# TengdaHan/DPC

Hardware: AMD Instinct MI355X
Metric: clips/sec (train step, B x8x3x5xHxW) (higher is better)
Workload: dtype bf16; 1 GPU; cfg2: resnet18 2d3d, img_dim 128, seq_len 5, num_seq 8, pred_step 3, batch 128/GPU, full train step (fwd+CE/top-k+bwd+all-reduce+Adam); global_batch=128, parallelism=dp1, init=reference init, random, launch=hipGraph replay, streams=2

## Files before the change

dpc_amd/csrc/conv_igemm_ws.hip:

```cpp
#include "conv_common.h"
#include <stdlib.h>

struct WsParams {
    GatherGeom g;
    const void* src;
    const void* wgt;
    void* out;
    const void* addend;
    float* stats;
    int Ncol, ldw, ldo;
    int gm, ntn, ntm;
    unsigned src_bytes, wgt_bytes;
    int tgroup, hw, nclip, tpt, cpkt;
    FastDiv d_hw;
    int plane;
    int parity;
    ParityInfo par;
    int dbg;
};
#ifdef DPC_WS_PROBE
#define WS_DBG(bit) (p.dbg & (bit))
#else
#define WS_DBG(bit) 0
#endif

#include "ws_frag.h"

template <bool HAS_ADD, bool PAR = false>
__global__ __launch_bounds__(512, 2) void igemm_ws_kernel(WsParams p) {
    typedef bf16_t T;
    typedef bf16_t TO;
    constexpr int BM = 256, BN = 128, BKE = 64;
    constexpr int STAGE = (BM + BN) * 128;
    constexpr int NST = 3;
    constexpr int EPO = 8, UPR = BN / EPO;
    __shared__ __attribute__((aligned(1024))) unsigned char lds[NST * STAGE];

    const GatherGeom& g = p.g;
    const int tid = threadIdx.x;
    const int lane = tid & 63;
#ifdef DPC_SIMT_EMU
    const int wv = tid >> 6;
#else
    const int wv = __builtin_amdgcn_readfirstlane(tid >> 6);
#endif
    const int n_tile = blockIdx.x / p.gm;
    const int m_prog = blockIdx.x % p.gm;
    const int nkc = g.Kp / BKE;
    const int my_tiles = (p.ntm - m_prog + p.gm - 1) / p.gm;
    struct ParCls { int j, rows, ct, ch, cw, Tc, Hc, Wc; FastDiv dT, dH, dW; };
    auto par_cls = [&](int mt) -> ParCls {
        ParCls k;
        int c;
        parity_tile(p.par, mt, c, k.j);
        k.cw = c & (g.sw - 1); k.ch = (c >> g.lsw) & (g.sh - 1); k.ct = c >> (g.lsw + g.lsh);
        k.Tc = k.ct ? p.par.dimc[0][1] : p.par.dimc[0][0]; k.dT = k.ct ? p.par.div[0][1] : p.par.div[0][0];
        k.Hc = k.ch ? p.par.dimc[1][1] : p.par.dimc[1][0]; k.dH = k.ch ? p.par.div[1][1] : p.par.div[1][0];
        k.Wc = k.cw ? p.par.dimc[2][1] : p.par.dimc[2][0]; k.dW = k.cw ? p.par.div[2][1] : p.par.div[2][0];
        k.rows = p.par.N * k.Tc * k.Hc * k.Wc;
        return k;
    };
    auto par_decode = [&](const ParCls& k, int lr, int& n, int& tq, int& hq, int& wq) {
        const unsigned q1 = fdiv((unsigned)lr, k.dW);
        wq = lr - (int)q1 * k.Wc;
        const unsigned q2 = fdiv(q1, k.dH);
        hq = (int)q1 - (int)q2 * k.Hc;
        const unsigned nn = fdiv(q2, k.dT);
        tq = (int)q2 - (int)nn * k.Tc;
        n = (int)nn;
    };
    auto par_row = [&](const ParCls& k, int r) -> int {
        const int lr = k.j * BM + r;
        if (lr >= k.rows) return g.M;
        int n, tq, hq, wq;
        par_decode(k, lr, n, tq, hq, wq);
        return (((n * g.RT + tq * g.st + k.ct) * g.RH + hq * g.sh + k.ch) * g.RW) + wq * g.sw + k.cw;
    };
    auto par_pk = [&](const ParCls& k, unsigned& pT, unsigned& pH, unsigned& pW) {
        pT = k.ct ? p.par.pk[0][1] : p.par.pk[0][0];
        pH = k.ch ? p.par.pk[1][1] : p.par.pk[1][0];
        pW = k.cw ? p.par.pk[2][1] : p.par.pk[2][0];
    };
    auto tile_row = [&](int mt, int r) -> int {
        if (!p.tgroup) return mt * BM + r;
        const int t = mt / p.tpt;
        const unsigned idx = (unsigned)((mt - t * p.tpt) * BM + r);
        const unsigned clip = fdiv(idx, p.d_hw);
        return (int)clip < p.nclip ? (int)((clip * (unsigned)g.RT + (unsigned)t) * (unsigned)p.hw + (idx - clip * (unsigned)p.hw)) : g.M;
    };
    auto tile_chunks = [&](int mt, int& lo, int& hi) {
        lo = 0; hi = nkc;
        if (PAR) {
            const ParCls k = par_cls(mt);
            unsigned pT, pH, pW;
            par_pk(k, pT, pH, pW);
            hi = par_pk_n(pT) * par_pk_n(pH) * par_pk_n(pW) * (g.Ci >> 6);
            return;
        }
        if (!p.tgroup) return;
        const int t = mt / p.tpt;
        int klo, khi;
        if (g.mode == 0) { klo = g.pt - t; khi = g.ST - 1 + g.pt - t; }
        else { klo = t + g.pt - (g.ST - 1); khi = t + g.pt; }
        if (klo < 0) klo = 0;
        if (khi > g.KT - 1) khi = g.KT - 1;
        lo = klo * p.cpkt; hi = (khi + 1) * p.cpkt;
    };
    int total = 0;
    for (int t = 0; t < my_tiles; ++t) {
        int lo, hi;
        tile_chunks(m_prog + t * p.gm, lo, hi);
        total += hi - lo;
    }
    const char* const zero = (const char*)dpc_zero16;

    if (wv >= 4) {
        const int lw = wv - 4;
        const int rl = lane >> 3;
        const int u = (lane & 7) ^ lds_swz1(8 * lw + rl);
        const BufRsrc rs_a = make_buf_rsrc(p.src, p.src_bytes);
        const BufRsrc rs_b = make_buf_rsrc(p.wgt, p.wgt_bytes);
        unsigned wrow[4];
        DPC_UNROLL
        for (int i = 0; i < 4; ++i) {
            const int n = n_tile * BN + 8 * (lw + 4 * i) + rl;
            wrow[i] = n < p.Ncol ? (unsigned)(n * p.ldw + u * 8) * 2u : DPC_BUF_OOB;
        }
        unsigned rowoff[8];
        unsigned vmask[8];
        auto range_bits = [](int x0, int sgn, int K, int S) -> unsigned {
            int lo, hi;
            if (sgn > 0) { lo = -x0; hi = S - 1 - x0; } else { lo = x0 - S + 1; hi = x0; }
            if (lo < 0) lo = 0;
            if (hi > K - 1) hi = K - 1;
            return hi >= lo ? (((2u << hi) - 1u) & ~((1u << lo) - 1u)) : 0u;
        };
        unsigned l_pT = 0, l_pH = 0, l_pW = 0;
        int l_jt = 0, l_jh = 0, l_jw = 0, l_cc = 0;
        auto decode_tile = [&](int mt) {
            const int mine = lane & 7;
            if (PAR) {
                const ParCls k = par_cls(mt);
                par_pk(k, l_pT, l_pH, l_pW);
                l_jt = l_jh = l_jw = l_cc = 0;
                const int lr = k.j * BM + 8 * (lw + 4 * mine) + rl;
                unsigned off = 0, m = 0;
                if (lr < k.rows) {
                    int n, tq, hq, wq;
                    par_decode(k, lr, n, tq, hq, wq);
                    off = (((((unsigned)(n * g.ST + tq) * (unsigned)g.SH + (unsigned)hq) * (unsigned)g.SW) + (unsigned)wq) * (unsigned)g.src_ld) * 2u;
                    DPC_UNROLL
                    for (int j = 0; j < 4; ++j) {
                        m |= (j < par_pk_n(l_pT) && (unsigned)(tq + par_pk_dl(l_pT, j)) < (unsigned)g.ST ? 1u : 0u) << j;
                        m |= (j < par_pk_n(l_pH) && (unsigned)(hq + par_pk_dl(l_pH, j)) < (unsigned)g.SH ? 1u : 0u) << (4 + j);
                        m |= (j < par_pk_n(l_pW) && (unsigned)(wq + par_pk_dl(l_pW, j)) < (unsigned)g.SW ? 1u : 0u) << (8 + j);
                    }
                }
                DPC_UNROLL
                for (int i = 0; i < 8; ++i) {
                    const int from = (lane & ~7) | i;
                    rowoff[i] = (unsigned)__shfl((int)off, from) + (unsigned)(u * 16);
                    vmask[i] = (unsigned)__shfl((int)m, from);
                }
                return;
            }
            const RowPos rp = decode_row(g, tile_row(mt, 8 * (lw + 4 * mine) + rl));
            const unsigned off = (((((unsigned)(rp.nbase + rp.t0) * (unsigned)g.SH + (unsigned)rp.h0) * (unsigned)g.SW) + (unsigned)rp.w0) *
                                  (unsigned)g.src_ld) * 2u;
            const int sgn = g.mode == 0 ? 1 : -1;
            const unsigned m = range_bits(rp.t0, sgn, g.KT, g.ST) | (range_bits(rp.h0, sgn, g.KH, g.SH) << g.KT) |
                               (range_bits(rp.w0, sgn, g.KW, g.SW) << (g.KT + g.KH));
            DPC_UNROLL
            for (int i = 0; i < 8; ++i) {
                const int from = (lane & ~7) | i;
                rowoff[i] = (unsigned)__shfl((int)off, from) + (unsigned)(u * 16);
                vmask[i] = (unsigned)__shfl((int)m, from);
            }
        };
        auto issue = [&](int kc, int stage) {
            unsigned char* st = lds + stage * STAGE;
            if (PAR) {
                const int jt = l_jt, jh = l_jh, jw = l_jw, cofs = l_cc * BKE;
                if (++l_cc == (g.Ci >> 6)) {
                    l_cc = 0;
                    if (++l_jw == par_pk_n(l_pW)) {
                        l_jw = 0;
                        if (++l_jh == par_pk_n(l_pH)) { l_jh = 0; ++l_jt; }
                    }
                }
                const int kt = par_pk_kl(l_pT, jt), kh = par_pk_kl(l_pH, jh), kw = par_pk_kl(l_pW, jw);
                const int dt = par_pk_dl(l_pT, jt), dh = par_pk_dl(l_pH, jh), dw = par_pk_dl(l_pW, jw);
                const unsigned sel = (1u << jt) | (1u << (4 + jh)) | (1u << (8 + jw));
                const unsigned tapoff = (unsigned)(((dt * g.SH + dh) * g.SW + dw) * g.src_ld + cofs) * 2u;
                const unsigned kd = (unsigned)(((kt * g.KH + kh) * g.KW + kw) * g.Ci + cofs);
                DPC_UNROLL
                for (int i = 0; i < 8; ++i) {
                    const bool ok = (vmask[i] & sel) == sel;
                    if (!WS_DBG(4 | 128)) glds16_buf(rs_a, ok ? rowoff[i] + tapoff : DPC_BUF_OOB, 0u, st + (lw + 4 * i) * 1024, lane);
                }
                DPC_UNROLL
                for (int i = 0; i < 4; ++i)
                    if (!WS_DBG(4 | 256)) glds16_buf(rs_b, wrow[i], kd * 2u, st + BM * 128 + (lw + 4 * i) * 1024, lane);
                return;
            }
            const int kd = kc * BKE;
            const int tap = (g.taps == 1) ? 0 : (kd >> g.log2C);
            const unsigned q = fdiv((unsigned)tap, g.dKW);
            const int kw = tap - (int)q * g.KW;
            const unsigned kt = fdiv(q, g.dKH);
            const int kh = (int)q - (int)kt * g.KH;
            const unsigned sel = (1u << kt) | (1u << (g.KT + kh)) | (1u << (g.KT + g.KH + kw));
            const int sgn = g.mode == 0 ? 1 : -1;
            const int cbase = (g.taps == 1) ? 0 : (tap << g.log2C);
            const unsigned tapoff = (unsigned)(sgn * ((((int)kt * g.SH + kh) * g.SW + kw) * g.src_ld) + (kd - cbase)) * 2u;
            DPC_UNROLL
            for (int i = 0; i < 8; ++i) {
                const bool ok = (vmask[i] & sel) == sel;
                if (!WS_DBG(4 | 128)) glds16_buf(rs_a, ok ? rowoff[i] + tapoff : DPC_BUF_OOB, 0u, st + (lw + 4 * i) * 1024, lane);
            }
            DPC_UNROLL
            for (int i = 0; i < 4; ++i)
                if (!WS_DBG(4 | 256)) glds16_buf(rs_b, wrow[i], (unsigned)kd * 2u, st + BM * 128 + (lw + 4 * i) * 1024, lane);
        };
        int it_tile = 0, it_kc = 0, it_hi = 0;
        bool it_new = true;
        auto issue_next = [&](int gc) {
            if (it_new) {
                const int mt = m_prog + it_tile * p.gm;
                decode_tile(mt);
                tile_chunks(mt, it_kc, it_hi);
                it_new = false;
            }
            issue(it_kc, gc % NST);
            if (++it_kc == it_hi) { it_new = true; ++it_tile; }
        };
        if (total > 0) issue_next(0);
        if (total > 1) issue_next(1);
        int kc_done = 0, cur_tile = 0, cur_n;
        {
            int lo, hi;
            tile_chunks(m_prog, lo, hi);
            cur_n = hi - lo;
        }
        for (int gc = 0; gc < total; ++gc) {
            if (gc + 1 < total) wait_vmcnt<12>(); else wait_vmcnt<0>();
            ws_barrier();
            if (gc + 2 < total) issue_next(gc + 2);
            if (++kc_done == cur_n) {
                kc_done = 0;
                ws_barrier();
                if (++cur_tile < my_tiles) {
                    int lo, hi;
                    tile_chunks(m_prog + cur_tile * p.gm, lo, hi);
                    cur_n = hi - lo;
                }
            }
        }
    }

    const int l31 = lane & 31, lhi = lane >> 5;
    const ldsa_t lds0 = ldsa(lds);
    const int fa0 = lds_unit_off(wv * 64 + l31, lhi);
    const int fb0 = BM * 128 + lds_unit_off(l31, lhi);
    const int cu = lane & 15, er = lane >> 4;
    const int col0 = n_tile * BN + cu * EPO;
    float s1[EPO], s2[EPO];
    DPC_UNROLL
    for (int e = 0; e < EPO; ++e) { s1[e] = 0.f; s2[e] = 0.f; }

    int gc = 0;
#ifndef DPC_SIMT_EMU
    __builtin_amdgcn_s_setprio(3);
#endif
    for (int t = 0; wv < 4 && t < my_tiles; ++t) {
        const int mt = m_prog + t * p.gm;
        ParCls ck = {};
        if (PAR) ck = par_cls(mt);
        int kc_lo, kc_hi;
        tile_chunks(mt, kc_lo, kc_hi);
        const int nkc_t = kc_hi - kc_lo;
        f32x16 acc[2][4];
        DPC_UNROLL
        for (int i = 0; i < 2; ++i)
            DPC_UNROLL
            for (int j = 0; j < 4; ++j)
                DPC_UNROLL
                for (int r = 0; r < 16; ++r) acc[i][j][r] = 0.f;
        u32x4 av0[8], av1[8];
        auto fetch_addend = [&](int i, u32x4 (&dst)[8]) {
            DPC_UNROLL
            for (int it = 0; it < 8; ++it) {
                const int row = PAR ? par_row(ck, wv * 64 + i * 32 + er + 4 * it) : tile_row(mt, wv * 64 + i * 32 + er + 4 * it);
                const bool ok = row < g.M && col0 < p.Ncol;
                const char* a = (const char*)p.addend + ((long long)row * p.ldo + col0) * 2;
                dst[it] = *(const u32x4*)(ok ? a : (const char*)p.addend);
            }
        };
        int stage_last = 0;
        {
            FragSet f0, f1;
            ws_barrier();
            ldsa_t pa = lds0 + (gc % NST) * STAGE + fa0, pb = lds0 + (gc % NST) * STAGE + fb0;
            frag_read_p2<4096>(f0, pa, pb);
            for (int kc = 0; kc < nkc_t; ++kc) {
                if (HAS_ADD && kc + 1 == nkc_t) fetch_addend(0, av0);
                step_il<true, 4096>(acc, f0, f1, pa ^ 32, pb ^ 32);
                step_il<true, 4096>(acc, f1, f0, pa ^ 64, pb ^ 64);
                step_il<true, 4096>(acc, f0, f1, pa ^ 96, pb ^ 96);
                frag_wait<0>(f1);
                ws_barrier();
                stage_last = gc % NST;
                ++gc;
                pa = lds0 + (gc % NST) * STAGE + fa0;
                pb = lds0 + (gc % NST) * STAGE + fb0;
                step_il<true, 4096>(acc, f1, f0, pa, pb);
            }
            WS_RETIRE_TAIL_READS(f0);
        }

        if (WS_DBG(2)) {
            if (acc[0][0][0] == 12345.f) *(float*)p.out = acc[1][3][5];
            continue;
        }
        unsigned char* mine = lds + stage_last * STAGE + wv * WS_STG_WAVE;
        DPC_UNROLL
        for (int i = 0; i < 2; ++i) {
            stage_block(mine, acc[i], l31, lhi);
            wave_lds_fence();
            if (HAS_ADD && i == 0) fetch_addend(1, av1);
            u32x4 ov[8];
            DPC_UNROLL
            for (int it = 0; it < 8; ++it) {
                const int row_l = er + 4 * it;
                ov[it] = *(const u32x4*)(mine + row_l * WS_STG_ROW + cu * EPO * 2);
            }
            wave_lds_fence();
            DPC_UNROLL
            for (int it = 0; it < 8; ++it) {
                const int row = PAR ? par_row(ck, wv * 64 + i * 32 + er + 4 * it) : tile_row(mt, wv * 64 + i * 32 + er + 4 * it);
                if (row < g.M && col0 < p.Ncol) {
                    u32x4 o = ov[it];
                    if (HAS_ADD) {
                        const u32x4 a = i == 0 ? av0[it] : av1[it];
                        float sv[EPO];
                        DPC_UNROLL
                        for (int e = 0; e < EPO; ++e) sv[e] = unit_get<TO>(o, e) + unit_get<TO>(a, e);
                        o = unit_pack<TO>(sv);
                    }
                    *(u32x4*)((char*)p.out + ((long long)row * p.ldo + col0) * 2) = o;
                    if (!HAS_ADD) {
                        DPC_UNROLL
                        for (int e = 0; e < EPO; ++e) {
                            const float v = unit_get<TO>(o, e);
                            s1[e] += v;
                            s2[e] += v * v;
                        }
                    }
                }
            }
        }
    }

    if (!HAS_ADD && p.stats) {
        DPC_UNROLL
        for (int e = 0; e < EPO; ++e) {
            s1[e] += __shfl_xor(s1[e], 16); s1[e] += __shfl_xor(s1[e], 32);
            s2[e] += __shfl_xor(s2[e], 16); s2[e] += __shfl_xor(s2[e], 32);
        }
        float* red = (float*)lds;
        __syncthreads();
        if (wv < 4 && lane < 16) {
            DPC_UNROLL
            for (int e = 0; e < EPO; ++e) {
                red[(wv * 2 + 0) * BN + cu * EPO + e] = s1[e];
                red[(wv * 2 + 1) * BN + cu * EPO + e] = s2[e];
            }
        }
        __syncthreads();
        if (tid < BN) {
            const int col = n_tile * BN + tid;
            if (col < p.Ncol) {
                float a = 0.f, b = 0.f;
                DPC_UNROLL
                for (int w = 0; w < 4; ++w) {
                    a += red[(w * 2 + 0) * BN + tid];
                    b += red[(w * 2 + 1) * BN + tid];
                }
                p.stats[((long long)m_prog * 2 + 0) * p.Ncol + col] = a;
                p.stats[((long long)m_prog * 2 + 1) * p.Ncol + col] = b;
            }
        }
    }
}


template <bool HAS_ADD>
__global__ __launch_bounds__(512, 2) void igemm_wsp_kernel(WsParams p) {
    typedef bf16_t TO;
    constexpr int BM = 256, BN = 128;
    constexpr int PWD = 18, NPP = PWD * PWD, NPIECE = (NPP + 7) / 8, PATCH = NPIECE * 1024;
    constexpr int BST = BN * 128, NSB = 4;
    constexpr int EPO = 8;
    constexpr int MAXP = (NPIECE + 3) / 4;
    static_assert(4 * WS_STG_WAVE <= PATCH, "epilogue staging fits a patch buffer");
    static_assert(2 * PATCH + NSB * BST <= 160 * 1024, "patches + ring fit the CU's LDS");
    __shared__ __attribute__((aligned(1024))) unsigned char lds[2 * PATCH + NSB * BST];
    unsigned char* const bring = lds + 2 * PATCH;

    const GatherGeom& g = p.g;
    const int tid = threadIdx.x;
    const int lane = tid & 63;
#ifdef DPC_SIMT_EMU
    const int wv = tid >> 6;
#else
    const int wv = __builtin_amdgcn_readfirstlane(tid >> 6);
#endif
    const int n_tile = blockIdx.x / p.gm;
    const int m_prog = blockIdx.x % p.gm;
    const int G = g.Ci >> 6;
    const int nkc = 9 * G;
    const int my_tiles = (p.ntm - m_prog + p.gm - 1) / p.gm;
    const int total = my_tiles * nkc;
    const char* const zero = (const char*)dpc_zero16;

    if (wv >= 4) {
        const int lw = wv - 4;
        const int rl = lane >> 3;
        const BufRsrc rs_a = make_buf_rsrc(p.src, p.src_bytes);
        const BufRsrc rs_b = make_buf_rsrc(p.wgt, p.wgt_bytes);
        const int ub = (lane & 7) ^ lds_swz1(8 * lw + rl);
        unsigned wrow[4];
        DPC_UNROLL
        for (int i = 0; i < 4; ++i) {
            const int n = n_tile * BN + 8 * (lw + 4 * i) + rl;
            wrow[i] = n < p.Ncol ? (unsigned)(n * p.ldw + ub * 8) * 2u : DPC_BUF_OOB;
        }
        unsigned poff[MAXP];
        DPC_UNROLL
        for (int i = 0; i < MAXP; ++i) {
            const int pp = 8 * (lw + 4 * i) + rl;
            const int pr = pp / PWD, pc = pp - pr * PWD;
            const bool ok = pp < NPP && pr >= 1 && pr <= 16 && pc >= 1 && pc <= 16;
            const int up = (lane & 7) ^ ((pc >> 1) & 7);
            poff[i] = ok ? (unsigned)((((pr - 1) * 16 + (pc - 1)) * g.src_ld + up * 8) * 2) : DPC_BUF_OOB;
        }
        const int n_mine = (NPIECE - lw + 3) / 4;
        int issued = 0;
        auto issue_patch = [&](int gg, int i0, int i1) {
            const int tl = gg / G, grp = gg - tl * G;
            const int mt = WS_DBG(512) ? m_prog & 7 : m_prog + tl * p.gm;
            const unsigned soff = (unsigned)((mt * BM * g.src_ld + grp * 64) * 2);
            unsigned char* dst = lds + (gg & 1) * PATCH;
            DPC_UNROLL
            for (int i = 0; i < MAXP; ++i)
                if (i >= i0 && i < i1 && i < n_mine && !WS_DBG(4 | 128)) {
                    glds16_buf(rs_a, poff[i], soff, dst + (lw + 4 * i) * 1024, lane);
                    ++issued;
                }
        };
        auto issue_b = [&](int gc) {
            const int gg = gc / 9, tap = gc - gg * 9;
            const int grp = gg % G;
            const int kd = tap * g.Ci + grp * 64;
            unsigned char* st = bring + (gc % NSB) * BST;
            if (WS_DBG(4 | 256)) return;
            DPC_UNROLL
            for (int i = 0; i < 4; ++i) glds16_buf(rs_b, wrow[i], (unsigned)kd * 2u, st + (lw + 4 * i) * 1024, lane);
            issued += 4;
        };
        if (total > 0) {
            issue_patch(0, 0, MAXP);
            issue_b(0);
        }
        issued = 0;
        if (total > 1) issue_b(1);
        int o2 = issued;
        issued = 0;
        if (total > 2) issue_b(2);
        int o1 = issued;
        for (int gc = 0; gc < total; ++gc) {
            wait_vmcnt_upto(o1 + o2);
            if (!WS_DBG(32)) ws_barrier();
            const int gg = gc / 9, q = gc - gg * 9;
            issued = 0;
            if (q < (MAXP + 1) / 2 && (gg + 1) * 9 < total) issue_patch(gg + 1, 2 * q, 2 * q + 2);
            if (gc + 3 < total) issue_b(gc + 3);
            o2 = o1;
            o1 = issued;
            if (q == 8 && (gg + 1) % G == 0) if (!WS_DBG(32)) ws_barrier();
        }
    }

    const int l31 = lane & 31, lhi = lane >> 5;
    int va[3];
    {
        const int pos0 = ((wv * 64 + l31) >> 4) * PWD + (l31 & 15);
        DPC_UNROLL
        for (int kw = 0; kw < 3; ++kw) {
            const int dw = g.mode == 0 ? kw : 2 - kw;
            const int p7 = (((l31 & 15) + dw) >> 1) & 7;
            va[kw] = (pos0 + dw) * 128 + ((lhi ^ p7) << 4);
        }
    }
    const ldsa_t lds0 = ldsa(lds);
    const int vb = lds_unit_off(l31, lhi);
    const int cu = lane & 15, er = lane >> 4;
    const int col0 = n_tile * BN + cu * EPO;
    float s1[EPO], s2[EPO];
    DPC_UNROLL
    for (int e = 0; e < EPO; ++e) { s1[e] = 0.f; s2[e] = 0.f; }

    int gc = 0;
#ifndef DPC_SIMT_EMU
    __builtin_amdgcn_s_setprio(3);
#endif
    for (int t = 0; wv < 4 && t < my_tiles; ++t) {
        const int mt = m_prog + t * p.gm;
        f32x16 acc[2][4];
        DPC_UNROLL
        for (int i = 0; i < 2; ++i)
            DPC_UNROLL
            for (int j = 0; j < 4; ++j)
                DPC_UNROLL
                for (int r = 0; r < 16; ++r) acc[i][j][r] = 0.f;
        u32x4 av0[8], av1[8];
        auto fetch_addend = [&](int i, u32x4 (&dst)[8]) {
            DPC_UNROLL
            for (int it = 0; it < 8; ++it) {
                const int row = mt * BM + wv * 64 + i * 32 + er + 4 * it;
                const bool ok = row < g.M && col0 < p.Ncol;
                const char* a = (const char*)p.addend + ((long long)row * p.ldo + col0) * 2;
                dst[it] = *(const u32x4*)(ok ? a : (const char*)p.addend);
            }
        };
        {
            FragSet f0, f1;
            if (!WS_DBG(32)) ws_barrier();
            ldsa_t a_row = lds0 + ((t * G) & 1) * PATCH + (g.mode == 0 ? 0 : 2) * (PWD * 128);
            ldsa_t b_st = lds0 + 2 * PATCH + (gc % NSB) * BST;
            ldsa_t pa = a_row + va[0];
            ldsa_t pb = b_st + vb;
            frag_read_p2<4608>(f0, pa, pb);
            for (int gk = 0; gk < 3 * G; ++gk) {
                const int grp = gk / 3, kh = gk - grp * 3;
                const bool last_gk = gk + 1 == 3 * G;
                const int kh_n = kh == 2 ? 0 : kh + 1, gg_n = t * G + (kh == 2 ? grp + 1 : grp);
                const ldsa_t a_row_n = lds0 + (gg_n & 1) * PATCH + (g.mode == 0 ? kh_n : 2 - kh_n) * (PWD * 128);
                static_for<3>([&](auto KWc) {
                    constexpr int KW = decltype(KWc)::value;
                    const bool last = last_gk && KW == 2;
                    if (HAS_ADD && last) fetch_addend(0, av0);
                    step_il<true, 4608>(acc, f0, f1, pa ^ 32, pb ^ 32);
                    step_il<true, 4608>(acc, f1, f0, pa ^ 64, pb ^ 64);
                    step_il<true, 4608>(acc, f0, f1, pa ^ 96, pb ^ 96);
                    frag_wait<0>(f1);
                    if (!WS_DBG(32)) ws_barrier();
                    ++gc;
                    b_st = lds0 + 2 * PATCH + (gc % NSB) * BST;
                    if (KW == 2) a_row = a_row_n;
                    pa = a_row + va[(KW + 1) % 3];
                    pb = b_st + vb;
                    step_il<true, 4608>(acc, f1, f0, pa, pb);
                });
            }
            WS_RETIRE_TAIL_READS(f0);
        }

        unsigned char* mine = lds + ((t * G + G - 1) & 1) * PATCH + wv * WS_STG_WAVE;
        if (WS_DBG(2)) {
            if (acc[0][0][0] == 12345.f) *(float*)p.out = acc[1][3][5];
            continue;
        }
        DPC_UNROLL
        for (int i = 0; i < 2; ++i) {
            stage_block(mine, acc[i], l31, lhi);
            wave_lds_fence();
            if (HAS_ADD && i == 0) fetch_addend(1, av1);
            u32x4 ov[8];
            DPC_UNROLL
            for (int it = 0; it < 8; ++it) {
                const int row_l = er + 4 * it;
                ov[it] = *(const u32x4*)(mine + row_l * WS_STG_ROW + cu * EPO * 2);
            }
            wave_lds_fence();
            DPC_UNROLL
            for (int it = 0; it < 8; ++it) {
                const int row = mt * BM + wv * 64 + i * 32 + er + 4 * it;
                if (row < g.M && col0 < p.Ncol && !WS_DBG(1)) {
                    u32x4 o = ov[it];
                    if (HAS_ADD) {
                        const u32x4 a = i == 0 ? av0[it] : av1[it];
                        float sv[EPO];
                        DPC_UNROLL
                        for (int e = 0; e < EPO; ++e) sv[e] = unit_get<TO>(o, e) + unit_get<TO>(a, e);
                        o = unit_pack<TO>(sv);
                    }
                    *(u32x4*)((char*)p.out + ((long long)row * p.ldo + col0) * 2) = o;
                    if (!HAS_ADD) {
                        DPC_UNROLL
                        for (int e = 0; e < EPO; ++e) {
                            const float v = unit_get<TO>(o, e);
                            s1[e] += v;
                            s2[e] += v * v;
                        }
                    }
                }
            }
        }
    }

    if (!HAS_ADD && p.stats) {
        DPC_UNROLL
        for (int e = 0; e < EPO; ++e) {
            s1[e] += __shfl_xor(s1[e], 16); s1[e] += __shfl_xor(s1[e], 32);
            s2[e] += __shfl_xor(s2[e], 16); s2[e] += __shfl_xor(s2[e], 32);
        }
        float* red = (float*)lds;
        __syncthreads();
        if (wv < 4 && lane < 16) {
            DPC_UNROLL
            for (int e = 0; e < EPO; ++e) {
                red[(wv * 2 + 0) * BN + cu * EPO + e] = s1[e];
                red[(wv * 2 + 1) * BN + cu * EPO + e] = s2[e];
            }
        }
        __syncthreads();
        if (tid < BN) {
            const int col = n_tile * BN + tid;
            if (col < p.Ncol) {
                float a = 0.f, b = 0.f;
                DPC_UNROLL
                for (int w = 0; w < 4; ++w) {
                    a += red[(w * 2 + 0) * BN + tid];
                    b += red[(w * 2 + 1) * BN + tid];
                }
                p.stats[((long long)m_prog * 2 + 0) * p.Ncol + col] = a;
                p.stats[((long long)m_prog * 2 + 1) * p.Ncol + col] = b;
            }
        }
    }
}


__global__ __launch_bounds__(512, 2) void igemm_wsd_kernel(WsParams p) {
    typedef bf16_t TO;
    constexpr int BM = 256, BN = 128;
    constexpr int PWD = 18, NPP = PWD * PWD, NPIECE = (NPP + 7) / 8, PATCH = NPIECE * 1024;
    constexpr int BST = BN * 128, NSB = 4;
    constexpr int EPO = 8;
    constexpr int MAXP = (NPIECE + 3) / 4;
    static_assert(4 * WS_STG_WAVE <= PATCH, "epilogue staging fits a patch buffer");
    static_assert(2 * PATCH + NSB * BST <= 160 * 1024, "patches + ring fit the CU's LDS");
    __shared__ __attribute__((aligned(1024))) unsigned char lds[2 * PATCH + NSB * BST];
    unsigned char* const bring = lds + 2 * PATCH;

    const GatherGeom& g = p.g;
    const int tid = threadIdx.x;
    const int lane = tid & 63;
#ifdef DPC_SIMT_EMU
    const int wv = tid >> 6;
#else
    const int wv = __builtin_amdgcn_readfirstlane(tid >> 6);
#endif
    const bool kindB = (int)blockIdx.x >= p.gm;
    const int m_prog = kindB ? (int)blockIdx.x - p.gm : (int)blockIdx.x;
    const int gmk = kindB ? p.ntn : p.gm;
    const int CPG = kindB ? 3 : 4;
    const int G = g.Ci >> 6;
    const int nkc = CPG * G;
    const int my_tiles = m_prog < p.ntm ? (p.ntm - m_prog + gmk - 1) / gmk : 0;
    const int total = my_tiles * nkc;
    const int py0 = 1, px0 = kindB ? 0 : 1, py1 = 0, px1 = kindB ? 1 : 0;
    auto shift_of = [&](int q, int& sy, int& sx) {
        if (kindB) { sy = q == 1; sx = q == 2; } else { sy = q >> 1; sx = q & 1; }
    };

    if (wv >= 4) {
        const int lw = wv - 4;
        const int rl = lane >> 3;
        const BufRsrc rs_a = make_buf_rsrc(p.src, p.src_bytes);
        const BufRsrc rs_b = make_buf_rsrc(p.wgt, p.wgt_bytes);
        const int ub = (lane & 7) ^ lds_swz1(8 * lw + rl);
        unsigned wrow[4];
        DPC_UNROLL
        for (int i = 0; i < 4; ++i) {
            const int n = 8 * (lw + 4 * (i & 1)) + rl;
            wrow[i] = (unsigned)(n * p.ldw + ub * 8) * 2u;
        }
        unsigned poff[MAXP];
        DPC_UNROLL
        for (int i = 0; i < MAXP; ++i) {
            const int pp = 8 * (lw + 4 * i) + rl;
            const int pr = pp / PWD, pc = pp - pr * PWD;
            const bool ok = pp < NPP && pr >= 1 && pr <= 16 && pc >= 1 && pc <= 16;
            const int up = (lane & 7) ^ ((pc >> 1) & 7);
            poff[i] = ok ? (unsigned)((((pr - 1) * 16 + (pc - 1)) * g.src_ld + up * 8) * 2) : DPC_BUF_OOB;
        }
        const int n_mine = (NPIECE - lw + 3) / 4;
        int issued = 0;
        auto issue_patch = [&](int gg, int i0, int i1) {
            const int tl = gg / G, grp = gg - tl * G;
            const int mt = m_prog + tl * gmk;
            const unsigned soff = (unsigned)((mt * BM * g.src_ld + grp * 64) * 2);
            unsigned char* dst = lds + (gg & 1) * PATCH;
            DPC_UNROLL
            for (int i = 0; i < MAXP; ++i)
                if (i >= i0 && i < i1 && i < n_mine) {
                    glds16_buf(rs_a, poff[i], soff, dst + (lw + 4 * i) * 1024, lane);
                    ++issued;
                }
        };
        auto issue_b = [&](int gc) {
            const int gg = gc / CPG, q = gc - gg * CPG;
            const int grp = gg % G;
            int sy, sx;
            shift_of(q, sy, sx);
            unsigned char* st = bring + (gc % NSB) * BST;
            DPC_UNROLL
            for (int i = 0; i < 4; ++i) {
                const int py = i < 2 ? py0 : py1, px = i < 2 ? px0 : px1;
                const bool valid = sy <= py && sx <= px;
                const int ky = py ? (sy ? 0 : 2) : 1, kx = px ? (sx ? 0 : 2) : 1;
                const unsigned kd = (unsigned)((ky * 3 + kx) * g.Ci + grp * 64);
                glds16_buf(rs_b, valid ? wrow[i] : DPC_BUF_OOB, kd * 2u, st + (lw + 4 * i) * 1024, lane);
            }
            issued += 4;
        };
        const int pslots = CPG - 2, ppc = (MAXP + pslots - 1) / pslots;
        if (total > 0) {
            issue_patch(0, 0, MAXP);
            issue_b(0);
        }
        issued = 0;
        if (total > 1) issue_b(1);
        int o2 = issued;
        issued = 0;
        if (total > 2) issue_b(2);
        int o1 = issued;
        for (int gc = 0; gc < total; ++gc) {
            wait_vmcnt_upto(o1 + o2);
            ws_barrier();
            const int gg = gc / CPG, q = gc - gg * CPG;
            issued = 0;
            if (q < pslots && (gg + 1) * CPG < total) issue_patch(gg + 1, ppc * q, ppc * q + ppc);
            if (gc + 3 < total) issue_b(gc + 3);
            o2 = o1;
            o1 = issued;
            if (q == CPG - 1 && (gg + 1) % G == 0) ws_barrier();
        }
        return;
    }

    const int l31 = lane & 31, lhi = lane >> 5;
    int va[2];
    {
        const int pos0 = ((wv * 64 + l31) >> 4) * PWD + (l31 & 15);
        DPC_UNROLL
        for (int sx = 0; sx < 2; ++sx) {
            const int dw = 1 + sx;
            const int p7 = (((l31 & 15) + dw) >> 1) & 7;
            va[sx] = (pos0 + dw) * 128 + ((lhi ^ p7) << 4);
        }
    }
    const ldsa_t lds0 = ldsa(lds);
    const int vb = lds_unit_off(l31, lhi);
    const int cu = lane & 15, er = lane >> 4;
    const int hpy = (cu >> 3) ? py1 : py0, hpx = (cu >> 3) ? px1 : px0;
    const int ccol = (cu & 7) * EPO;

    int gc = 0;
#ifndef DPC_SIMT_EMU
    __builtin_amdgcn_s_setprio(3);
#endif
    for (int t = 0; t < my_tiles; ++t) {
        const int mt = m_prog + t * gmk;
        f32x16 acc[2][4];
        DPC_UNROLL
        for (int i = 0; i < 2; ++i)
            DPC_UNROLL
            for (int j = 0; j < 4; ++j)
                DPC_UNROLL
                for (int r = 0; r < 16; ++r) acc[i][j][r] = 0.f;
        {
            FragSet f0, f1;
            ws_barrier();
            int grp = 0, q = 0;
            ldsa_t a_pat = lds0 + ((t * G) & 1) * PATCH;
            ldsa_t pa = a_pat + PWD * 128 + va[0];
            ldsa_t pb = lds0 + 2 * PATCH + (gc % NSB) * BST + vb;
            frag_read_p2<4608>(f0, pa, pb);
            for (int c = 0; c < nkc; ++c) {
                step_il<true, 4608>(acc, f0, f1, pa ^ 32, pb ^ 32);
                step_il<true, 4608>(acc, f1, f0, pa ^ 64, pb ^ 64);
                step_il<true, 4608>(acc, f0, f1, pa ^ 96, pb ^ 96);
                frag_wait<0>(f1);
                ws_barrier();
                ++gc;
                if (++q == CPG) { q = 0; ++grp; }
                int sy, sx;
                shift_of(q, sy, sx);
                a_pat = lds0 + ((t * G + grp) & 1) * PATCH;
                pa = a_pat + (1 + sy) * (PWD * 128) + (sx ? va[1] : va[0]);
                pb = lds0 + 2 * PATCH + (gc % NSB) * BST + vb;
                step_il<true, 4608>(acc, f1, f0, pa, pb);
            }
            WS_RETIRE_TAIL_READS(f0);
        }

        unsigned char* mine = lds + ((t * G + G - 1) & 1) * PATCH + wv * WS_STG_WAVE;
        DPC_UNROLL
        for (int i = 0; i < 2; ++i) {
            stage_block(mine, acc[i], l31, lhi);
            wave_lds_fence();
            u32x4 ov[8];
            DPC_UNROLL
            for (int it = 0; it < 8; ++it) {
                const int row_l = er + 4 * it;
                ov[it] = *(const u32x4*)(mine + row_l * WS_STG_ROW + cu * EPO * 2);
            }
            wave_lds_fence();
            DPC_UNROLL
            for (int it = 0; it < 8; ++it) {
                const int r = wv * 64 + i * 32 + er + 4 * it;
                const int a = r >> 4, b = r & 15;
                const long long orow = ((long long)mt * g.RH + 2 * a + hpy) * g.RW + 2 * b + hpx;
                if (mt < p.ntm) *(u32x4*)((char*)p.out + (orow * p.ldo + ccol) * 2) = ov[it];
            }
        }
    }
}

static int env_int(const char* name, int dflt) {
    const char* e = getenv(name);
    return e ? atoi(e) : dflt;
}
static int ws_enabled() { static int v = env_int("DPC_IGEMM_WS", 1); return v; }
static int ws_min_rows() { static int v = env_int("DPC_IGEMM_WS_MINROWS", 256 * 64); return v; }
static int ws_max_programs() { static int v = env_int("DPC_IGEMM_WS_GM", 256); return v; }

static bool ws_plan(const dpc_conv_desc* d, WsParams* p) {
    if (!ws_enabled()) return false;
    if (d->dtype_in != DPC_BF16 || d->dtype_out != DPC_BF16) return false;
    if (d->Co < 64 || d->Co % 8 || d->ldo % 8 || d->ldw % 8) return false;
    GatherGeom& g = p->g;
    if (make_gather_geom(d, &g)) return false;
    if (g.Kp % 64 || (g.taps > 1 && g.Ci % 64)) return false;
    const bool unit_strides = g.st == 1 && g.sh == 1 && g.sw == 1;
    const bool fits32 = (long long)(g.M / (g.RT * g.RH * g.RW)) * g.ST * g.SH * g.SW * g.src_ld < (1ll << 30);
    if (!fits32 || g.KT + g.KH + g.KW > 32) return false;
    p->parity = 0;
    int par_tiles = 0;
    if (!(g.mode == 0 || unit_strides)) {
        static const int par_on = env_int("DPC_IGEMM_WS_PAR", 1);
        if (!par_on || g.taps == 1 || !dpc_plan_parity(g, p->par, 64, 256, false, &par_tiles)) return false;
        if (!p->par.pk_ok) return false;
        for (int c = 0; c < p->par.ncls; ++c)
            if (p->par.cnt[0][c / (g.sw * g.sh)] * p->par.cnt[1][(c / g.sw) % g.sh] * p->par.cnt[2][c % g.sw] == 0) return false;
        p->parity = 1;
    }
    static const int par_min_co = env_int("DPC_IGEMM_WS_PAR_MINCO", 128);
    if (d->Co < (p->parity ? par_min_co : 128)) return false;
    if (g.M < ws_min_rows()) return false;
    p->Ncol = d->Co; p->ldw = d->ldw; p->ldo = d->ldo;
    const long long wbytes = ((long long)(d->Co - 1) * d->ldw + g.Kp) * 2;
    if (wbytes >= (1ll << 31)) return false;
    p->src_bytes = (unsigned)((long long)(g.M / (g.RT * g.RH * g.RW)) * g.ST * g.SH * g.SW * g.src_ld * 2);
    p->wgt_bytes = (unsigned)wbytes;
    p->ntn = (d->Co + 127) / 128;
    p->ntm = p->parity ? par_tiles : (g.M + 255) / 256;
    p->tgroup = 0; p->hw = 1; p->nclip = 0; p->tpt = 1; p->cpkt = 1; p->d_hw = make_fastdiv(1);
    {
        static const int plane_on = env_int("DPC_IGEMM_WS_PLANE", 1);
        p->plane = !p->parity && plane_on && g.KT == 1 && g.KH == 3 && g.KW == 3 && g.pt == 0 && g.ph == 1 && g.pw == 1 && unit_strides && g.RT == g.ST &&
                   g.RH == 16 && g.RW == 16 && g.SH == 16 && g.SW == 16 && g.Ci % 64 == 0;
    }
    {
        static const int tg_on = env_int("DPC_IGEMM_WS_TGROUP", 1);
        const int hw = g.RH * g.RW;
        if (tg_on && !p->parity && g.KT > 1 && unit_strides && g.RT == g.ST && g.RT > 1) {
            p->tgroup = 1; p->hw = hw; p->d_hw = make_fastdiv((uint32_t)hw);
            p->nclip = g.M / (g.RT * hw);
            p->tpt = (int)(((long long)p->nclip * hw + 255) / 256);
            p->cpkt = g.KH * g.KW * (g.Ci / 64);
            p->ntm = g.RT * p->tpt;
        }
    }
    int gm = dpc_persistent_grid(ws_max_programs()) / p->ntn;
    if (gm < 1) gm = 1;
    if (gm > p->ntm) gm = p->ntm;
    if (gm >= 8) gm &= ~7;
    p->gm = gm;
    if (p->parity) dpc_parity_rounds(p->par, gm);
    return true;
}

static bool wsd_plan(const dpc_conv_desc* d, WsParams* p) {
    static const int on = env_int("DPC_IGEMM_WSD", 1);
    if (!on || !ws_enabled()) return false;
    if (d->dtype_in != DPC_BF16 || d->dtype_out != DPC_BF16 || d->mode != 1) return false;
    if (d->KT != 1 || d->KH != 3 || d->KW != 3 || d->st != 1 || d->sh != 2 || d->sw != 2 || d->pt != 0 || d->ph != 1 || d->pw != 1) return false;
    if (d->RT != d->ST || d->SH != 16 || d->SW != 16 || d->RH != 32 || d->RW != 32) return false;
    if (d->Ci != 128 || d->src_ld != 128 || d->Co != 64 || d->ldo % 8 || d->ldo < 64 || d->ldw % 8 || d->ldw < 9 * 128) return false;
    GatherGeom& g = p->g;
    if (make_gather_geom(d, &g)) return false;
    const long long planes = (long long)d->N * d->RT;
    if (planes * 256 * 128 * 2 >= (1ll << 30) || planes * 1024 * (long long)d->ldo * 2 >= (1ll << 40)) return false;
    static const int min_planes = env_int("DPC_WSD_MINPLANES", 512);
    if (planes < min_planes) return false;
    p->parity = 0; p->plane = 0; p->tgroup = 0; p->hw = 1; p->nclip = 0; p->tpt = 1; p->cpkt = 1; p->d_hw = make_fastdiv(1);
    p->Ncol = d->Co; p->ldw = d->ldw; p->ldo = d->ldo;
    p->src_bytes = (unsigned)(planes * 256 * 128 * 2);
    p->wgt_bytes = (unsigned)(((long long)(d->Co - 1) * d->ldw + 9 * 128) * 2);
    p->ntm = (int)planes;
    static const int a_share = env_int("DPC_WSD_A_PERMILLE", 556);
    const int wgs = dpc_persistent_grid(ws_max_programs());
    int gma = (int)((long long)wgs * a_share / 1000);
    if (gma < 1) gma = 1;
    if (gma > wgs - 1) gma = wgs - 1;
    p->gm = gma;
    p->ntn = wgs - gma;
    return wgs >= 2;
}

int dpc_conv_ws_rows(const dpc_conv_desc* d) {
    WsParams p;
    if (!d || !ws_plan(d, &p)) return 0;
    return p.gm;
}

int dpc_conv_ws_try(const dpc_conv_desc* d, const void* src, const void* wgt, void* out, const void* addend, float* stats,
                    const EpiExtra& epi, hipStream_t stream) {
    WsParams p;
    if (!addend && !stats && !epi_any(epi) && wsd_plan(d, &p)) {
        if (((uintptr_t)out % 16) || ((uintptr_t)src % 16) || ((uintptr_t)wgt % 16)) return 1;
        p.src = src; p.wgt = wgt; p.out = out; p.addend = nullptr; p.stats = nullptr; p.dbg = 0;
        DPC_LAUNCH(igemm_wsd_kernel, dim3((unsigned)(p.gm + p.ntn)), dim3(512), stream, p);
        return dpc_launch_status();
    }
    if (!ws_plan(d, &p)) return 1;
    if (epi_any(epi)) return 1;
    if (addend && stats) return 1;
    if (p.parity && (addend || stats)) return 1;
    if (((uintptr_t)out % 16) || ((uintptr_t)addend % 16) || ((uintptr_t)src % 16) || ((uintptr_t)wgt % 16)) return 1;
    p.src = src; p.wgt = wgt; p.out = out; p.addend = addend; p.stats = stats;
#ifdef DPC_WS_PROBE
    p.dbg = getenv("DPC_WS_DBG") ? atoi(getenv("DPC_WS_DBG")) : 0;
#else
    p.dbg = 0;
#endif
    dim3 grid((unsigned)(p.gm * p.ntn)), block(512);
    if (p.parity) {
        DPC_LAUNCH((igemm_ws_kernel<false, true>), grid, block, stream, p);
    } else if (p.plane) {
        if (addend) {
            DPC_LAUNCH((igemm_wsp_kernel<true>), grid, block, stream, p);
        } else {
            DPC_LAUNCH((igemm_wsp_kernel<false>), grid, block, stream, p);
        }
    } else if (addend) {
        DPC_LAUNCH((igemm_ws_kernel<true>), grid, block, stream, p);
    } else {
        DPC_LAUNCH((igemm_ws_kernel<false>), grid, block, stream, p);
    }
    return dpc_launch_status();
}
```

Before: 5035 clips/s.

## Fuse backward BN/ReLU-mask epilogue into warp-specialized implicit-GEMM conv kernels

Adds an EPI template path to the warp-specialized igemm kernels so conv launches that carry an extra epilogue (addend mask, BN-backward reduction using raw activations, mean/invstd, and masks) run on the ws kernels instead of falling back. The epilogue loads, masks and per-column stat reductions now happen inside the GEMM epilogue, with partial sums kept in extra LDS. This removes separate elementwise/reduction passes and lets these convs use the faster ws kernels. In exchange it raises register and LDS pressure in the kernels, which may lower occupancy, and it can be turned off with DPC_WS_EPI=0.

```diff
diff --git a/dpc_amd/csrc/conv_igemm_ws.hip b/dpc_amd/csrc/conv_igemm_ws.hip
--- a/dpc_amd/csrc/conv_igemm_ws.hip
+++ b/dpc_amd/csrc/conv_igemm_ws.hip
@@ -17,6 +17,13 @@
     int parity;
     ParityInfo par;
     int dbg;
+    EpiExtra epi;
+};
+
+constexpr int WS_EPI_LDS = 4 * 16 * 16 * 4;
+struct WsEpiOps {
+    u32x4 raw[8];
+    unsigned ab[8], bb[8];
 };
 #ifdef DPC_WS_PROBE
 #define WS_DBG(bit) (p.dbg & (bit))
@@ -26,7 +33,64 @@
 
 #include "ws_frag.h"
 
-template <bool HAS_ADD, bool PAR = false>
+template <class RowF>
+__device__ __forceinline__ void ws_epi_fetch_raw(const WsParams& p, int col0, RowF row, u32x4 (&dst)[8]) {
+    DPC_UNROLL
+    for (int it = 0; it < 8; ++it) {
+        const int r = row(it);
+        const bool ok = r < p.g.M && col0 < p.Ncol;
+        const char* a = (const char*)p.epi.bn_raw + ((long long)r * p.ldo + col0) * 2;
+        dst[it] = *(const u32x4*)(ok ? a : (const char*)p.epi.bn_raw);
+    }
+}
+template <bool ADD, class RowF>
+__device__ __forceinline__ void ws_epi_fetch_bits(const WsParams& p, int col0, RowF row, unsigned (&bits)[8]) {
+    DPC_UNROLL
+    for (int it = 0; it < 8; ++it) {
+        const int r = row(it);
+        const long long u = (r < p.g.M && col0 < p.Ncol) ? ((long long)r * p.ldo + col0) >> 3 : 0ll;
+        const unsigned ab = (ADD && p.epi.addend_mask) ? (unsigned)p.epi.addend_mask[u] : 0xffu;
+        const unsigned bb = p.epi.bn_mask ? (unsigned)p.epi.bn_mask[u] : 0xffu;
+        bits[it] = ab | (bb << 8);
+    }
+}
+__device__ __forceinline__ void ws_epi_coefs(const WsParams& p, int col0, bool bnred, float (&mu)[8], float (&is)[8]) {
+    DPC_UNROLL
+    for (int e = 0; e < 8; ++e) {
+        const bool ok = bnred && col0 < p.Ncol;
+        mu[e] = ok ? p.epi.bn_mean[col0 + e] : 0.f;
+        is[e] = ok ? p.epi.bn_invstd[col0 + e] : 0.f;
+    }
+}
+__device__ __forceinline__ void ws_epi_flush(float* esum, int wv, int lane, float (&e1)[8], float (&e2)[8]) {
+    DPC_UNROLL
+    for (int e = 0; e < 8; ++e) {
+        e1[e] += __shfl_xor(e1[e], 16); e1[e] += __shfl_xor(e1[e], 32);
+        e2[e] += __shfl_xor(e2[e], 16); e2[e] += __shfl_xor(e2[e], 32);
+    }
+    if (lane < 16) {
+        float* r = esum + (wv * 16 + lane) * 16;
+        DPC_UNROLL
+        for (int e = 0; e < 8; ++e) { r[e] += e1[e]; r[8 + e] += e2[e]; }
+    }
+}
+__device__ __forceinline__ void ws_epi_stats(const WsParams& p, const float* esum, int tid, int n_tile, int m_prog) {
+    if (tid < 128) {
+        const int col = n_tile * 128 + tid;
+        if (col < p.Ncol) {
+            float a = 0.f, b = 0.f;
+            DPC_UNROLL
+            for (int w = 0; w < 4; ++w) {
+                a += esum[(w * 16 + (tid >> 3)) * 16 + (tid & 7)];
+                b += esum[(w * 16 + (tid >> 3)) * 16 + 8 + (tid & 7)];
+            }
+            p.stats[((long long)m_prog * 2 + 0) * p.Ncol + col] = a;
+            p.stats[((long long)m_prog * 2 + 1) * p.Ncol + col] = b;
+        }
+    }
+}
+
+template <bool HAS_ADD, bool PAR = false, int EPI = 0>
 __global__ __launch_bounds__(512, 2) void igemm_ws_kernel(WsParams p) {
     typedef bf16_t T;
     typedef bf16_t TO;
@@ -34,7 +98,8 @@
     constexpr int STAGE = (BM + BN) * 128;
     constexpr int NST = 3;
     constexpr int EPO = 8, UPR = BN / EPO;
-    __shared__ __attribute__((aligned(1024))) unsigned char lds[NST * STAGE];
+    static_assert(!(EPI && PAR), "the parity-class tiles take no fused epilogue");
+    __shared__ __attribute__((aligned(1024))) unsigned char lds[NST * STAGE + (EPI ? WS_EPI_LDS : 0)];
 
     const GatherGeom& g = p.g;
     const int tid = threadIdx.x;
@@ -267,6 +332,12 @@
     float s1[EPO], s2[EPO];
     DPC_UNROLL
     for (int e = 0; e < EPO; ++e) { s1[e] = 0.f; s2[e] = 0.f; }
+    constexpr bool bnred = EPI == 1;
+    float* const esum = (float*)(lds + NST * STAGE);
+    if (EPI && wv < 4 && lane < 16) {
+        DPC_UNROLL
+        for (int e = 0; e < 16; ++e) esum[(wv * 16 + lane) * 16 + e] = 0.f;
+    }
 
     int gc = 0;
 #ifndef DPC_SIMT_EMU
@@ -296,6 +367,12 @@
                 dst[it] = *(const u32x4*)(ok ? a : (const char*)p.addend);
             }
         };
+        u32x4 rv0[8], rv1[8];
+        unsigned eb0[8], eb1[8];
+        float mu[EPO], is[EPO], e1[EPO], e2[EPO];
+        auto ep_row = [&](int i, int it) -> int {
+            return PAR ? par_row(ck, wv * 64 + i * 32 + er + 4 * it) : tile_row(mt, wv * 64 + i * 32 + er + 4 * it);
+        };
         int stage_last = 0;
         {
             FragSet f0, f1;
@@ -304,6 +381,7 @@
             frag_read_p2<4096>(f0, pa, pb);
             for (int kc = 0; kc < nkc_t; ++kc) {
                 if (HAS_ADD && kc + 1 == nkc_t) fetch_addend(0, av0);
+                if (EPI && !HAS_ADD && kc + 1 == nkc_t) ws_epi_fetch_raw(p, col0, [&](int it) { return ep_row(0, it); }, rv0);
                 step_il<true, 4096>(acc, f0, f1, pa ^ 32, pb ^ 32);
                 step_il<true, 4096>(acc, f1, f0, pa ^ 64, pb ^ 64);
                 step_il<true, 4096>(acc, f0, f1, pa ^ 96, pb ^ 96);
@@ -323,11 +401,32 @@
             continue;
         }
         unsigned char* mine = lds + stage_last * STAGE + wv * WS_STG_WAVE;
+        if (EPI) {
+            DPC_UNROLL
+            for (int e = 0; e < EPO; ++e) { e1[e] = 0.f; e2[e] = 0.f; }
+        }
         DPC_UNROLL
         for (int i = 0; i < 2; ++i) {
             stage_block(mine, acc[i], l31, lhi);
             wave_lds_fence();
-            if (HAS_ADD && i == 0) fetch_addend(1, av1);
+            if (HAS_ADD && !EPI && i == 0) fetch_addend(1, av1);
+            if (EPI) {
+                auto row0 = [&](int it) { return ep_row(0, it); };
+                auto row1 = [&](int it) { return ep_row(1, it); };
+                if (i == 0) {
+                    if (HAS_ADD && bnred) ws_epi_fetch_raw(p, col0, row0, rv0);
+                    ws_epi_fetch_bits<HAS_ADD>(p, col0, row0, eb0);
+                    ws_epi_coefs(p, col0, bnred, mu, is);
+                    if (!HAS_ADD) {
+                        ws_epi_fetch_raw(p, col0, row1, rv1);
+                        ws_epi_fetch_bits<HAS_ADD>(p, col0, row1, eb1);
+                    }
+                } else if (HAS_ADD) {
+                    fetch_addend(1, av1);
+                    if (bnred) ws_epi_fetch_raw(p, col0, row1, rv1);
+                    ws_epi_fetch_bits<HAS_ADD>(p, col0, row1, eb1);
+                }
+            }
             u32x4 ov[8];
             DPC_UNROLL
             for (int it = 0; it < 8; ++it) {
@@ -340,7 +439,11 @@
                 const int row = PAR ? par_row(ck, wv * 64 + i * 32 + er + 4 * it) : tile_row(mt, wv * 64 + i * 32 + er + 4 * it);
                 if (row < g.M && col0 < p.Ncol) {
                     u32x4 o = ov[it];
-                    if (HAS_ADD) {
+                    if (EPI) {
+                        const unsigned eb = i == 0 ? eb0[it] : eb1[it];
+                        epi_unit<TO, EPO>(o, HAS_ADD, i == 0 ? av0[it] : av1[it], eb & 0xffu, bnred, i == 0 ? rv0[it] : rv1[it], eb >> 8,
+                                          mu, is, e1, e2);
+                    } else if (HAS_ADD) {
                         const u32x4 a = i == 0 ? av0[it] : av1[it];
                         float sv[EPO];
                         DPC_UNROLL
@@ -348,7 +451,7 @@
                         o = unit_pack<TO>(sv);
                     }
                     *(u32x4*)((char*)p.out + ((long long)row * p.ldo + col0) * 2) = o;
-                    if (!HAS_ADD) {
+                    if (!HAS_ADD && !EPI) {
                         DPC_UNROLL
                         for (int e = 0; e < EPO; ++e) {
                             const float v = unit_get<TO>(o, e);
@@ -359,9 +462,14 @@
                 }
             }
         }
-    }
-
-    if (!HAS_ADD && p.stats) {
+        if (EPI) ws_epi_flush(esum, wv, lane, e1, e2);
+    }
+
+    if (EPI && p.stats) {
+        __syncthreads();
+        ws_epi_stats(p, esum, tid, n_tile, m_prog);
+    }
+    if (!EPI && !HAS_ADD && p.stats) {
         DPC_UNROLL
         for (int e = 0; e < EPO; ++e) {
             s1[e] += __shfl_xor(s1[e], 16); s1[e] += __shfl_xor(s1[e], 32);
@@ -394,7 +502,7 @@
 }
 
 
-template <bool HAS_ADD>
+template <bool HAS_ADD, int EPI = 0>
 __global__ __launch_bounds__(512, 2) void igemm_wsp_kernel(WsParams p) {
     typedef bf16_t TO;
     constexpr int BM = 256, BN = 128;
@@ -403,8 +511,8 @@
     constexpr int EPO = 8;
     constexpr int MAXP = (NPIECE + 3) / 4;
     static_assert(4 * WS_STG_WAVE <= PATCH, "epilogue staging fits a patch buffer");
-    static_assert(2 * PATCH + NSB * BST <= 160 * 1024, "patches + ring fit the CU's LDS");
-    __shared__ __attribute__((aligned(1024))) unsigned char lds[2 * PATCH + NSB * BST];
+    static_assert(2 * PATCH + NSB * BST + WS_EPI_LDS <= 160 * 1024, "patches + ring (+ EPI sums) fit the CU's LDS");
+    __shared__ __attribute__((aligned(1024))) unsigned char lds[2 * PATCH + NSB * BST + (EPI ? WS_EPI_LDS : 0)];
     unsigned char* const bring = lds + 2 * PATCH;
 
     const GatherGeom& g = p.g;
@@ -509,6 +617,12 @@
     float s1[EPO], s2[EPO];
     DPC_UNROLL
     for (int e = 0; e < EPO; ++e) { s1[e] = 0.f; s2[e] = 0.f; }
+    constexpr bool bnred = EPI == 1;
+    float* const esum = (float*)(lds + 2 * PATCH + NSB * BST);
+    if (EPI && wv < 4 && lane < 16) {
+        DPC_UNROLL
+        for (int e = 0; e < 16; ++e) esum[(wv * 16 + lane) * 16 + e] = 0.f;
+    }
 
     int gc = 0;
 #ifndef DPC_SIMT_EMU
@@ -516,6 +630,11 @@
 #endif
     for (int t = 0; wv < 4 && t < my_tiles; ++t) {
         const int mt = m_prog + t * p.gm;
+        u32x4 rv0[8], rv1[8];
+        unsigned eb0[8], eb1[8];
+        float mu[EPO], is[EPO], e1[EPO], e2[EPO];
+        auto row0 = [&](int it) { return mt * BM + wv * 64 + er + 4 * it; };
+        auto row1 = [&](int it) { return mt * BM + wv * 64 + 32 + er + 4 * it; };
         f32x16 acc[2][4];
         DPC_UNROLL
         for (int i = 0; i < 2; ++i)
@@ -550,6 +669,7 @@
                     constexpr int KW = decltype(KWc)::value;
                     const bool last = last_gk && KW == 2;
                     if (HAS_ADD && last) fetch_addend(0, av0);
+                    if (EPI && !HAS_ADD && last) ws_epi_fetch_raw(p, col0, row0, rv0);
                     step_il<true, 4608>(acc, f0, f1, pa ^ 32, pb ^ 32);
                     step_il<true, 4608>(acc, f1, f0, pa ^ 64, pb ^ 64);
                     step_il<true, 4608>(acc, f0, f1, pa ^ 96, pb ^ 96);
@@ -571,11 +691,30 @@
             if (acc[0][0][0] == 12345.f) *(float*)p.out = acc[1][3][5];
             continue;
         }
+        if (EPI) {
+            DPC_UNROLL
+            for (int e = 0; e < EPO; ++e) { e1[e] = 0.f; e2[e] = 0.f; }
+        }
         DPC_UNROLL
         for (int i = 0; i < 2; ++i) {
             stage_block(mine, acc[i], l31, lhi);
             wave_lds_fence();
-            if (HAS_ADD && i == 0) fetch_addend(1, av1);
+            if (HAS_ADD && !EPI && i == 0) fetch_addend(1, av1);
+            if (EPI) {
+                if (i == 0) {
+                    if (HAS_ADD && bnred) ws_epi_fetch_raw(p, col0, row0, rv0);
+                    ws_epi_fetch_bits<HAS_ADD>(p, col0, row0, eb0);
+                    ws_epi_coefs(p, col0, bnred, mu, is);
+                    if (!HAS_ADD) {
+                        ws_epi_fetch_raw(p, col0, row1, rv1);
+                        ws_epi_fetch_bits<HAS_ADD>(p, col0, row1, eb1);
+                    }
+                } else if (HAS_ADD) {
+                    fetch_addend(1, av1);
+                    if (bnred) ws_epi_fetch_raw(p, col0, row1, rv1);
+                    ws_epi_fetch_bits<HAS_ADD>(p, col0, row1, eb1);
+                }
+            }
             u32x4 ov[8];
             DPC_UNROLL
             for (int it = 0; it < 8; ++it) {
@@ -588,7 +727,11 @@
                 const int row = mt * BM + wv * 64 + i * 32 + er + 4 * it;
                 if (row < g.M && col0 < p.Ncol && !WS_DBG(1)) {
                     u32x4 o = ov[it];
-                    if (HAS_ADD) {
+                    if (EPI) {
+                        const unsigned eb = i == 0 ? eb0[it] : eb1[it];
+                        epi_unit<TO, EPO>(o, HAS_ADD, i == 0 ? av0[it] : av1[it], eb & 0xffu, bnred, i == 0 ? rv0[it] : rv1[it], eb >> 8,
+                                          mu, is, e1, e2);
+                    } else if (HAS_ADD) {
                         const u32x4 a = i == 0 ? av0[it] : av1[it];
                         float sv[EPO];
                         DPC_UNROLL
@@ -596,7 +739,7 @@
                         o = unit_pack<TO>(sv);
                     }
                     *(u32x4*)((char*)p.out + ((long long)row * p.ldo + col0) * 2) = o;
-                    if (!HAS_ADD) {
+                    if (!HAS_ADD && !EPI) {
                         DPC_UNROLL
                         for (int e = 0; e < EPO; ++e) {
                             const float v = unit_get<TO>(o, e);
@@ -607,9 +750,14 @@
                 }
             }
         }
-    }
-
-    if (!HAS_ADD && p.stats) {
+        if (EPI) ws_epi_flush(esum, wv, lane, e1, e2);
+    }
+
+    if (EPI && p.stats) {
+        __syncthreads();
+        ws_epi_stats(p, esum, tid, n_tile, m_prog);
+    }
+    if (!EPI && !HAS_ADD && p.stats) {
         DPC_UNROLL
         for (int e = 0; e < EPO; ++e) {
             s1[e] += __shfl_xor(s1[e], 16); s1[e] += __shfl_xor(s1[e], 32);
@@ -933,23 +1081,44 @@
     WsParams p;
     if (!addend && !stats && !epi_any(epi) && wsd_plan(d, &p)) {
         if (((uintptr_t)out % 16) || ((uintptr_t)src % 16) || ((uintptr_t)wgt % 16)) return 1;
-        p.src = src; p.wgt = wgt; p.out = out; p.addend = nullptr; p.stats = nullptr; p.dbg = 0;
+        p.src = src; p.wgt = wgt; p.out = out; p.addend = nullptr; p.stats = nullptr; p.dbg = 0; p.epi = epi_none();
         DPC_LAUNCH(igemm_wsd_kernel, dim3((unsigned)(p.gm + p.ntn)), dim3(512), stream, p);
         return dpc_launch_status();
     }
     if (!ws_plan(d, &p)) return 1;
-    if (epi_any(epi)) return 1;
-    if (addend && stats) return 1;
-    if (p.parity && (addend || stats)) return 1;
+    const bool ex = epi_any(epi);
+    if (ex) {
+        static const int epi_on = env_int("DPC_WS_EPI", 1);
+        if (!epi_on || p.parity) return 1;
+    } else {
+        if (addend && stats) return 1;
+        if (p.parity && (addend || stats)) return 1;
+    }
     if (((uintptr_t)out % 16) || ((uintptr_t)addend % 16) || ((uintptr_t)src % 16) || ((uintptr_t)wgt % 16)) return 1;
-    p.src = src; p.wgt = wgt; p.out = out; p.addend = addend; p.stats = stats;
+    p.src = src; p.wgt = wgt; p.out = out; p.addend = addend; p.stats = stats; p.epi = epi;
 #ifdef DPC_WS_PROBE
     p.dbg = getenv("DPC_WS_DBG") ? atoi(getenv("DPC_WS_DBG")) : 0;
 #else
     p.dbg = 0;
 #endif
     dim3 grid((unsigned)(p.gm * p.ntn)), block(512);
-    if (p.parity) {
+    if (ex) {
+        if (p.plane) {
+            if (!epi.bn_raw) {
+                DPC_LAUNCH((igemm_wsp_kernel<true, 2>), grid, block, stream, p);
+            } else if (addend) {
+                DPC_LAUNCH((igemm_wsp_kernel<true, 1>), grid, block, stream, p);
+            } else {
+                DPC_LAUNCH((igemm_wsp_kernel<false, 1>), grid, block, stream, p);
+            }
+        } else if (!epi.bn_raw) {
+            DPC_LAUNCH((igemm_ws_kernel<true, false, 2>), grid, block, stream, p);
+        } else if (addend) {
+            DPC_LAUNCH((igemm_ws_kernel<true, false, 1>), grid, block, stream, p);
+        } else {
+            DPC_LAUNCH((igemm_ws_kernel<false, false, 1>), grid, block, stream, p);
+        }
+    } else if (p.parity) {
         DPC_LAUNCH((igemm_ws_kernel<false, true>), grid, block, stream, p);
     } else if (p.plane) {
         if (addend) {
```

Result: slower. 4968 clips/s, median of 2 (-1.3%).
